# DavidPeicho/loupiote

Measured on AMD Instinct MI355X. Metric: Mrays/s (+ ms/frame) at 1920×1080, 4 spp, Sponza; 1/2/4/8 GPU, higher is better.
Workload: dtype f32

## Files before the change

bindings/rust/loupiote_hip/src/ffi.rs:

```rust
#![allow(non_camel_case_types, non_upper_case_globals, dead_code)]
use std::os::raw::{c_char, c_int, c_uint, c_void};

pub const LPT_ABI_VERSION: u32 = 6;
pub const LPT_INVALID_INDEX: u32 = 0xFFFFFFFF;
pub const LPT_PUNCTUAL_POINT: u32 = 0;
pub const LPT_PUNCTUAL_SPOT: u32 = 1;
pub const LPT_PUNCTUAL_DIRECTIONAL: u32 = 2;
pub const LPT_ALPHA_OPAQUE: u32 = 0;
pub const LPT_ALPHA_MASK: u32 = 1;
pub const LPT_ACCEL_BUILD_HOST_SAH: u32 = 0;
pub const LPT_ACCEL_BUILD_GPU_LBVH: u32 = 1;
pub const LPT_UPLOAD_NO_TEXTURE_PAIRS: u32 = 0x100;
pub const LPT_COMM_ID_BYTES: u32 = 128;
pub const LPT_OK: c_int = 0;
pub const LPT_ERR_FILE_NOT_FOUND: c_int = 1;
pub const LPT_ERR_READBACK: c_int = 2;
pub const LPT_ERR_ACCEL_BUILD: c_int = 3;
pub const LPT_ERR_HIP: c_int = 4;
pub const LPT_ERR_RCCL: c_int = 5;
pub const LPT_ERR_INVALID_ARG: c_int = 6;
pub const LPT_BLIT_PATHTRACE: c_int = 0;
pub const LPT_BLIT_DENOISED: c_int = 1;
pub const LPT_BLIT_TEMPORAL: c_int = 2;
pub const LPT_BLIT_GBUFFER: c_int = 3;
// ... 8 lines not shown
pub const LPT_OPT_TAIL_LANES: c_int = 5;
pub const LPT_OPT_EXPERIMENT_BASE: c_int = 256;
pub const LPT_EXP_PIPE_RAYS: c_int = 0;
pub const LPT_EXP_REFILL: c_int = 1;
pub const LPT_EXP_TRACE_WAVES_PER_CU: c_int = 2;
pub const LPT_EXP_SHADE_BLOCKS_PER_CU: c_int = 3;
pub const LPT_EXP_PATH_WAVES_PER_CU: c_int = 4;
pub const LPT_EXP_PATH_REFILL: c_int = 5;
pub const LPT_EXP_OCC_CELL_MILLI: c_int = 6;
pub const LPT_EXP_STEP_BUDGET: c_int = 7;
pub const LPT_EXP_BUDGET_RAYS: c_int = 8;
pub const LPT_EXP_PACKET_QUADS: c_int = 9;
pub const LPT_EXP_SPLIT_RAYS: c_int = 10;
pub const LPT_EXP_BUDGET_SPLIT: c_int = 11;
pub const LPT_EXP_LANE_PHASE: c_int = 12;

#[repr(C)] pub struct lpt_device { _private: [u8; 0] }
#[repr(C)] pub struct lpt_scene { _private: [u8; 0] }
#[repr(C)] pub struct lpt_scene_gpu { _private: [u8; 0] }
#[repr(C)] pub struct lpt_probe { _private: [u8; 0] }
#[repr(C)] pub struct lpt_renderer { _private: [u8; 0] }
#[repr(C)] pub struct lpt_comm { _private: [u8; 0] }
#[repr(C)] pub struct lpt_host_frame { _private: [u8; 0] }

#[repr(C)] #[derive(Copy, Clone, Debug)]
pub struct lpt_material {
    pub color: [f32; 4],
    pub roughness: f32,
    pub reflectivity: f32,
    pub albedo_texture: u32,
// ... 220 lines not shown
```

include/lpt.h:

```cpp
#ifndef LPT_H
#define LPT_H

#include <stddef.h>
#include <stdint.h>

#ifdef __cplusplus
extern "C" {
#endif

#define LPT_ABI_VERSION 6u

#define LPT_INVALID_INDEX 0xFFFFFFFFu

enum {
    LPT_OK = 0,
    LPT_ERR_FILE_NOT_FOUND = 1,
    LPT_ERR_READBACK = 2,
    LPT_ERR_ACCEL_BUILD = 3,
    LPT_ERR_HIP = 4,
    LPT_ERR_RCCL = 5,
    LPT_ERR_INVALID_ARG = 6
};

const char *lpt_last_error(void);
// ... 274 lines not shown
} lpt_option;
#define LPT_OPT_EXPERIMENT(name) (LPT_OPT_EXPERIMENT_BASE + (name))
typedef enum lpt_experiment {
    LPT_EXP_PIPE_RAYS = 0,
    LPT_EXP_REFILL = 1,
    LPT_EXP_TRACE_WAVES_PER_CU = 2,
    LPT_EXP_SHADE_BLOCKS_PER_CU = 3,
    LPT_EXP_PATH_WAVES_PER_CU = 4,
    LPT_EXP_PATH_REFILL = 5,
    LPT_EXP_OCC_CELL_MILLI = 6,
    LPT_EXP_STEP_BUDGET = 7,
    LPT_EXP_BUDGET_RAYS = 8,
    LPT_EXP_PACKET_QUADS = 9,
    LPT_EXP_SPLIT_RAYS = 10,
    LPT_EXP_BUDGET_SPLIT = 11,
    LPT_EXP_LANE_PHASE = 12
} lpt_experiment;
int lpt_renderer_set_option(lpt_renderer *r, int option, uint64_t value);
int lpt_renderer_get_option(const lpt_renderer *r, int option, uint64_t *value);
int lpt_shard_layout(uint32_t width, uint32_t height, uint32_t tile_w, uint32_t tile_h, uint32_t world_size, uint32_t rank,
                     uint32_t *out_slots, uint32_t *out_slot_offset);
int lpt_shard_layout_weighted(uint32_t width, uint32_t height, uint32_t tile_w, uint32_t tile_h, uint32_t world_size, uint32_t rank,
                              const uint32_t *weights_or_null, uint32_t *out_slots, uint32_t *out_slot_offset);
int lpt_shard_owner(uint32_t world_size, const uint32_t *weights_or_null, uint32_t tile, uint32_t *out_rank);
int lpt_renderer_get_ray_counts(lpt_renderer *r, lpt_ray_counts *out);
int lpt_renderer_get_queue_counts(lpt_renderer *r, uint32_t *closest, uint32_t *shadow, uint32_t cap);
int lpt_renderer_reset_ray_counts(lpt_renderer *r);
int lpt_renderer_get_step_histogram(lpt_renderer *r, uint32_t *max_steps, uint32_t *hist12);
int lpt_renderer_enable_stats(lpt_renderer *r, int flag);
int lpt_renderer_synchronize(lpt_renderer *r);
int lpt_renderer_stream(lpt_renderer *r, void **hip_stream);
// ... 6 lines not shown
```

loupiote_amd/_abi.py:

```python
import ctypes as C
import os

import numpy as np

_HERE = os.path.dirname(os.path.abspath(__file__))
LIB_PATH = os.environ.get("LPT_LIB_PATH") or os.path.join(_HERE, "libloupiote_hip.so")

LPT_OK = 0
LPT_ERR_FILE_NOT_FOUND = 1
LPT_ERR_READBACK = 2
LPT_ERR_ACCEL_BUILD = 3
LPT_ERR_HIP = 4
LPT_ERR_RCCL = 5
LPT_ERR_INVALID_ARG = 6
COMM_ID_BYTES = 128
OPT_EXPERIMENT_BASE = 256
OPTIONS = {"packet_primary": 1, "wavefront_rays": 2, "path_rays": 3, "coop_rays": 4, "tail_lanes": 5}
EXPERIMENTS = {"pipe_rays": 0, "refill": 1, "trace_waves_per_cu": 2, "shade_blocks_per_cu": 3, "path_waves_per_cu": 4, "path_refill": 5, "occ_cell_milli": 6,
               "step_budget": 7, "budget_rays": 8, "packet_quads": 9, "split_rays": 10, "budget_split": 11, "lane_phase": 12}
OPTIONS.update({k: OPT_EXPERIMENT_BASE + v for k, v in EXPERIMENTS.items()})
EXCHANGE_GATHER_TILES = 0
HOST_FRAME_HOST_ONLY = 1
EXCHANGE_REDUCE = 1
INVALID_INDEX = 0xFFFFFFFF
LIGHT_BIT = 0x80000000

MATERIAL_DT = np.dtype([("color", "<f4", 4), ("roughness", "<f4"), ("reflectivity", "<f4"),
                        ("albedo_texture", "<u4"), ("mra_texture", "<u4")])
VERTEX_DT = np.dtype([("position", "<f4", 4), ("normal", "<f4", 4)])
LIGHT_DT = np.dtype([("normal", "<f4", 4), ("tangent", "<f4", 4), ("bitangent", "<f4", 4), ("origin", "<f4", 4)])
PUNCTUAL_DT = np.dtype([("position", "<f4", 4), ("direction", "<f4", 4), ("color", "<f4", 4), ("cone", "<f4", 4)])
PUNCTUAL_POINT, PUNCTUAL_SPOT, PUNCTUAL_DIRECTIONAL = 0, 1, 2
ALPHA_OPAQUE, ALPHA_MASK = 0, 1
INSTANCE_DT = np.dtype([("model_to_world", "<f4", 16), ("blas_index", "<u4"), ("material_index", "<u4"),
# ... 181 lines not shown
```

loupiote_amd/csrc/device.hip:

```cpp
#include <hip/hip_runtime.h>

#include <dlfcn.h>

#include <algorithm>
#include <cmath>
#include <map>
#include <memory>
#include <cstdlib>
#include <functional>
#include <mutex>
#include <new>
#include <numeric>

#include "common.h"
#include "env_dist.h"
#include "kernels.h"
#include "build_kernels.h"
#include <hipcub/hipcub.hpp>
#include <rccl/rccl.h>

using namespace lpt;
using namespace lptd;

#define TRY(expr) do { const int st__ = (expr); if (st__ != LPT_OK) return st__; } while (0)
// ... 171 lines not shown
    uint32_t max_bounces = 3, user_seed = 0;
    int env_sampling = 0;
    float vfov = 0.78539816339744830962f;
    uint32_t rank = 0, world = 1, tile_w = 32, tile_h = 8;
    std::vector<uint32_t> weights;
    ShardMap map{1u, 1u, {0u}};
    ShardTable h_table{};
    std::vector<uint32_t> h_offset;
    ShardTable *d_table = nullptr;
    bool use_noise = false, stats = false, timings = false;
    int refill = 44;
    int sort_queues = 0;
    uint32_t shade_blocks_per_cu = 0;
    uint32_t trace_waves_per_cu = 0;
    uint32_t lane_phase = 1;
    uint32_t n_slots = 0;
    float4 *accum = nullptr, *scratch = nullptr;
    lpt_comm *comm = nullptr;
    float4 *frame = nullptr, *xstage = nullptr;
    size_t xstage_elems = 0;
    bool presented = false;
    hipEvent_t xevent = nullptr;
    bool xevent_recorded = false;
    Totals *totals = nullptr;
    uint32_t step_budget = kStepBudget, budget_rays = kBudgetRays;
    bool budget_split = false;
    uint32_t coop_rays = kCoopRays;
    uint32_t tail_lanes = 4u;
    uint64_t split_rays = kSplitRays;
    uint32_t *err_host = nullptr, *err_dev = nullptr;
// ... 1032 lines not shown
    HIP_TRY(hipMalloc(&wf.sq.o, sizeof(float4) * n));
    HIP_TRY(hipMalloc(&wf.sq.d, sizeof(float4) * n));
    HIP_TRY(hipMalloc(&wf.sq.c, sizeof(float4) * n));
    HIP_TRY(hipMalloc(&wf.hits, sizeof(float4) * n));
    HIP_TRY(hipMalloc(&wf.Lsum, sizeof(float4) * n));
    HIP_TRY(hipMalloc(&wf.strag, sizeof(uint32_t) * 2 * n));
    wf.ray_cap = n;
    return LPT_OK;
}

static int ensure_lane(lpt_renderer *r, int l) {
    Wavefront &wf = r->wf[l];
    if (l > 0 && !wf.stream) HIP_TRY(hipStreamCreateWithFlags(&wf.stream, hipStreamNonBlocking));
    if (!wf.done) HIP_TRY(hipEventCreateWithFlags(&wf.done, hipEventDisableTiming));
    if (!wf.consumed) HIP_TRY(hipEventCreateWithFlags(&wf.consumed, hipEventDisableTiming));
    if (!wf.ctr) HIP_TRY(hipMalloc(&wf.ctr, sizeof(FrameCounters)));
    return LPT_OK;
}

static int alloc_frame_buffers(lpt_renderer *r) {
    HIP_TRY(hipSetDevice(r->dev->ordinal));
    HIP_TRY(hipStreamSynchronize(r->stream));
    free_frame_buffers(r);
    if (!r->w || !r->h) return LPT_OK;
    uint32_t tiles_x, n_tiles, n_slots;
    shard_geometry(r, tiles_x, n_tiles, n_slots);
    const size_t px = (size_t)r->w * r->h;
    r->n_slots = n_slots;
    if (r->rank == 0u) {
        r->h_table = make_shard_table(r->weights, r->world, n_tiles, r->tile_w * r->tile_h, r->h_offset);
        if (!r->d_table) HIP_TRY(hipMalloc(&r->d_table, sizeof(ShardTable)));
// ... 257 lines not shown
    case LPT_OPT_EXPERIMENT(LPT_EXP_PIPE_RAYS): r->pipe_rays = (uint32_t)std::min<uint64_t>(value, 0x7FFFFFFFu); break;
    case LPT_OPT_WAVEFRONT_RAYS: r->wavefront_rays = std::max<uint64_t>(value, 64u); break;
    case LPT_OPT_EXPERIMENT(LPT_EXP_REFILL): if (value > 63u) return fail(LPT_ERR_INVALID_ARG, "LPT_EXP_REFILL: 0..63"); r->refill = (int)value; break;
    case LPT_OPT_EXPERIMENT(LPT_EXP_TRACE_WAVES_PER_CU): if (value > 32u) return fail(LPT_ERR_INVALID_ARG, "LPT_EXP_TRACE_WAVES_PER_CU: 0 (auto) or 1..32"); r->trace_waves_per_cu = (uint32_t)value; break;
    case LPT_OPT_EXPERIMENT(LPT_EXP_SHADE_BLOCKS_PER_CU): if (value > 64u) return fail(LPT_ERR_INVALID_ARG, "LPT_EXP_SHADE_BLOCKS_PER_CU: 0 (by the submission) or 1..64"); r->shade_blocks_per_cu = (uint32_t)value; break;
    case LPT_OPT_PATH_RAYS: r->path_rays = (uint32_t)std::min<uint64_t>(value, 0x7FFFFFFFu); break;
    case LPT_OPT_EXPERIMENT(LPT_EXP_PATH_WAVES_PER_CU): if (value < 1u || value > 32u) return fail(LPT_ERR_INVALID_ARG, "LPT_EXP_PATH_WAVES_PER_CU: 1..32"); r->path_waves_per_cu = (uint32_t)value; break;
    case LPT_OPT_EXPERIMENT(LPT_EXP_PATH_REFILL): if (value > 63u) return fail(LPT_ERR_INVALID_ARG, "LPT_EXP_PATH_REFILL: 0..63"); r->path_refill = (int)value; break;
    case LPT_OPT_EXPERIMENT(LPT_EXP_OCC_CELL_MILLI): r->occ_cell = (float)std::min<uint64_t>(value, 1000000u) * 1.0e-3f; break;
    case LPT_OPT_EXPERIMENT(LPT_EXP_STEP_BUDGET): r->step_budget = (uint32_t)std::min<uint64_t>(value, 1u << 20); break;
    case LPT_OPT_EXPERIMENT(LPT_EXP_BUDGET_RAYS): r->budget_rays = (uint32_t)std::min<uint64_t>(value, 0x7FFFFFFFu); break;
    case LPT_OPT_EXPERIMENT(LPT_EXP_PACKET_QUADS): r->packet_quads = value != 0; break;
    case LPT_OPT_EXPERIMENT(LPT_EXP_SPLIT_RAYS): r->split_rays = value; break;
    case LPT_OPT_EXPERIMENT(LPT_EXP_BUDGET_SPLIT): r->budget_split = value != 0; break;
    case LPT_OPT_EXPERIMENT(LPT_EXP_LANE_PHASE): if (value > 2u) return fail(LPT_ERR_INVALID_ARG, "LPT_EXP_LANE_PHASE: 0 (free), 1 (offset start), 2 (alternating traversal)"); r->lane_phase = (uint32_t)value; break;
    case LPT_OPT_TAIL_LANES: r->tail_lanes = (uint32_t)std::min<uint64_t>(value, kTailMax); break;
    case LPT_OPT_COOP_RAYS: r->coop_rays = (uint32_t)std::min<uint64_t>(value, 0x7FFFFFFFu); break;
    default: return fail(LPT_ERR_INVALID_ARG, "lpt_renderer_set_option: unknown option %d", option);
    }
    return LPT_OK;
}
int lpt_renderer_get_option(const lpt_renderer *r, int option, uint64_t *value) {
    if (!r || !value) return fail(LPT_ERR_INVALID_ARG, "lpt_renderer_get_option: null");
    switch (option) {
    case LPT_OPT_PACKET_PRIMARY: *value = r->packet_primary; break;
    case LPT_OPT_EXPERIMENT(LPT_EXP_PIPE_RAYS): *value = r->pipe_rays; break;
    case LPT_OPT_WAVEFRONT_RAYS: *value = r->wavefront_rays; break;
    case LPT_OPT_EXPERIMENT(LPT_EXP_REFILL): *value = (uint64_t)r->refill; break;
    case LPT_OPT_EXPERIMENT(LPT_EXP_TRACE_WAVES_PER_CU): *value = r->trace_waves_per_cu; break;
    case LPT_OPT_EXPERIMENT(LPT_EXP_SHADE_BLOCKS_PER_CU): *value = r->shade_blocks_per_cu; break;
    case LPT_OPT_PATH_RAYS: *value = r->path_rays; break;
    case LPT_OPT_EXPERIMENT(LPT_EXP_PATH_WAVES_PER_CU): *value = r->path_waves_per_cu; break;
    case LPT_OPT_EXPERIMENT(LPT_EXP_PATH_REFILL): *value = (uint64_t)r->path_refill; break;
    case LPT_OPT_EXPERIMENT(LPT_EXP_OCC_CELL_MILLI): *value = (uint64_t)(r->occ_cell * 1000.0f + 0.5f); break;
    case LPT_OPT_EXPERIMENT(LPT_EXP_STEP_BUDGET): *value = r->step_budget; break;
    case LPT_OPT_EXPERIMENT(LPT_EXP_BUDGET_RAYS): *value = r->budget_rays; break;
    case LPT_OPT_EXPERIMENT(LPT_EXP_PACKET_QUADS): *value = r->packet_quads; break;
    case LPT_OPT_EXPERIMENT(LPT_EXP_SPLIT_RAYS): *value = r->split_rays; break;
    case LPT_OPT_EXPERIMENT(LPT_EXP_BUDGET_SPLIT): *value = r->budget_split; break;
    case LPT_OPT_EXPERIMENT(LPT_EXP_LANE_PHASE): *value = r->lane_phase; break;
    case LPT_OPT_TAIL_LANES: *value = r->tail_lanes; break;
    case LPT_OPT_COOP_RAYS: *value = r->coop_rays; break;
    default: return fail(LPT_ERR_INVALID_ARG, "lpt_renderer_get_option: unknown option %d", option);
    }
    return LPT_OK;
}
int lpt_renderer_enable_stats(lpt_renderer *r, int flag) {
    if (!r) return fail(LPT_ERR_INVALID_ARG, "lpt_renderer_enable_stats: null");
    FLUSH_OR_RETURN(r);
    r->stats = flag != 0;
    if (flag) {
        HIP_TRY(hipSetDevice(r->dev->ordinal));
        if (!r->occ_table) HIP_TRY(hipMalloc(&r->occ_table, sizeof(uint32_t) * kOccEntries));
        HIP_TRY(hipMemsetAsync(r->occ_table, 0, sizeof(uint32_t) * kOccEntries, r->stream));
        HIP_TRY(hipStreamSynchronize(r->stream));
// ... 183 lines not shown
        const uint32_t trace_blocks = std::min<uint32_t>(div_up(n_rays, kTraceBlock), waves);
        const size_t lds = stack_bytes(sc);
        const bool dense = (r->w % r->tile_w == 0u) && (r->h % r->tile_h == 0u);

        const float pixel_rad = 2.0f * th / (float)std::max(r->h, 1u);
        const bool packet = !masked && (r->packet_primary == 1u || (r->packet_primary == 2u && pixel_rad <= kPacketMaxPixelRad));
        tk.packet = packet;
        OccProbe occ{nullptr, 0u, 0.0f};
        if (!masked && r->stats && r->occ_table && r->occ_cell > 0.0f) occ = OccProbe{r->occ_table, kOccEntries - 1u, 1.0f / r->occ_cell};
        const bool tail_launch = !masked && !r->stats && (solo || r->budget_split) && n_rays <= r->budget_rays;
        const uint32_t tail = tail_launch ? std::min(std::min(r->tail_lanes, kTailMax), (uint32_t)std::max(r->refill, 0)) : 0u;
        const uint32_t budget = (tail_launch && !tail && r->step_budget) ? r->step_budget : 0u;
        const size_t tail_lds = tail ? sizeof(uint32_t) * tail_lds_words(r->sg->stats.max_depth) : 0u;
        const bool coop_all = !masked && !r->stats && r->coop_rays && n_rays <= r->coop_rays;
        const bool path = !masked && r->path_rays && n_rays <= r->path_rays && !coop_all;
        const int slot = cur_slot(r);
        Wavefront *w = &wf;
        tk.stages = nb + 1u;
        tk.run = [=](uint32_t t, const PhaseHooks &ph) -> int {
            if (ph.wait_start) HIP_TRY(hipStreamWaitEvent(s, ph.wait_start, 0));
            auto trace = [&](int cb, int sb) {
                stage_begin(r, cb >= 0 ? ST_INTERSECT : ST_SHADOW, s, slot);
                const Queue qin = w->q[(uint32_t)(cb < 0 ? 0 : cb) & 1u];
                const int launch_no = cb >= 0 ? cb : (int)nb;
                if (coop_all) {
                    const size_t clds = sizeof(uint32_t) * coop_stack_entries(kCoopStack, r->sg->stats.max_depth);
                    hipLaunchKernelGGL(k_trace_coop<false>, dim3(std::min(2u * n_rays, cus * kCoopWavesPerCu)), dim3(kTraceBlock), clds, s, sc, qin, w->hits, w->sq, w->Lsum, w->ctr, cb, sb, (const uint32_t *)nullptr, launch_no);
                    stage_end(r, s, slot);
                    return;
                }
// ... 7 lines not shown
                    if (pipe) hipLaunchKernelGGL((k_trace<false, true, true>), dim3(trace_blocks), dim3(kTraceBlock), lds + tail_lds, s, TraceKernargs{sc, qin, w->hits, w->sq, w->Lsum, w->ctr, cb, sb, r->refill, occ, 0u, w->strag, launch_no, tail});
                    else hipLaunchKernelGGL((k_trace<false, false, true>), dim3(trace_blocks), dim3(kTraceBlock), lds + tail_lds, s, TraceKernargs{sc, qin, w->hits, w->sq, w->Lsum, w->ctr, cb, sb, r->refill, occ, 0u, w->strag, launch_no, tail});
                } else if (pipe) {
                    if (r->stats) hipLaunchKernelGGL((k_trace<true, true>), dim3(trace_blocks), dim3(kTraceBlock), lds + 64u, s, TraceKernargs{sc, qin, w->hits, w->sq, w->Lsum, w->ctr, cb, sb, r->refill, occ, budget, w->strag, launch_no, 0u});
                    else hipLaunchKernelGGL((k_trace<false, true>), dim3(trace_blocks), dim3(kTraceBlock), lds, s, TraceKernargs{sc, qin, w->hits, w->sq, w->Lsum, w->ctr, cb, sb, r->refill, occ, budget, w->strag, launch_no, 0u});
                } else if (r->stats) hipLaunchKernelGGL((k_trace<true, false>), dim3(trace_blocks), dim3(kTraceBlock), lds + 64u, s, TraceKernargs{sc, qin, w->hits, w->sq, w->Lsum, w->ctr, cb, sb, r->refill, occ, budget, w->strag, launch_no, 0u});
                else hipLaunchKernelGGL((k_trace<false, false>), dim3(trace_blocks), dim3(kTraceBlock), lds, s, TraceKernargs{sc, qin, w->hits, w->sq, w->Lsum, w->ctr, cb, sb, r->refill, occ, budget, w->strag, launch_no, 0u});
                if (budget) {
                    const size_t clds = sizeof(uint32_t) * coop_stack_entries(kCoopStack, r->sg->stats.max_depth);
                    if (r->stats) hipLaunchKernelGGL(k_trace_coop<true>, dim3(cus * kCoopWavesPerCu), dim3(kTraceBlock), clds, s, sc, qin, w->hits, w->sq, w->Lsum, w->ctr, cb, sb, w->strag, launch_no);
                    else hipLaunchKernelGGL(k_trace_coop<false>, dim3(cus * kCoopWavesPerCu), dim3(kTraceBlock), clds, s, sc, qin, w->hits, w->sq, w->Lsum, w->ctr, cb, sb, w->strag, launch_no);
                }
                stage_end(r, s, slot);
            };
            if (t == 0u) {
                HIP_TRY(hipMemsetAsync(w->ctr, 0, sizeof(FrameCounters), s));
                stage_begin(r, ST_RAYGEN, s, slot);
                if (dense) {
                    hipLaunchKernelGGL(k_raygen<true>, dim3(stream_blocks), dim3(kBlock), 0, s, p, nz, w->q[0], w->Lsum, w->ctr);
                } else {
                    hipLaunchKernelGGL(k_raygen<false>, dim3(stream_blocks), dim3(kBlock), 0, s, p, nz, w->q[0], w->Lsum, w->ctr);
                }
                stage_end(r, s, slot);
                if (ph.wait_trav) HIP_TRY(hipStreamWaitEvent(s, ph.wait_trav, 0));
                if (packet) {
                    stage_begin(r, ST_PRIMARY, s, slot);
                    const uint32_t packets = div_up(n_rays, 64u);
                    const size_t plds = (size_t)(48u + 7u * r->sg->stats.max_depth + 8u) * sizeof(uint32_t);
                    const uint32_t quad_slots = (r->packet_quads && dense && p.block8 && p.n_slots % 64u == 0u && p.slot0 % 64u == 0u && n_samples % 4u == 0u) ? p.n_slots : 0u;
                    if (r->stats) hipLaunchKernelGGL(k_trace_packet<true>, dim3(std::min(packets, cus * kPacketBlocksPerCu)), dim3(kTraceBlock), plds, s, sc, w->q[0], w->hits, w->ctr, 0, quad_slots);
                    else hipLaunchKernelGGL(k_trace_packet<false>, dim3(std::min(packets, cus * kPacketBlocksPerCu)), dim3(kTraceBlock), plds, s, sc, w->q[0], w->hits, w->ctr, 0, quad_slots);
                    stage_end(r, s, slot);
                } else if (coop_all || !path) trace(0, -1);
                if (path) {
                    stage_begin(r, ST_PATH, s, slot);
                    const uint32_t pblocks = std::min<uint32_t>(div_up(n_rays, kTraceBlock), std::max(8u, (cus * r->path_waves_per_cu) & ~7u));
                    const size_t plds = lds + kPathLdsExtra;
                    auto launch_path = [&](auto G, auto S, auto P) {
                        constexpr bool g = decltype(G)::value, st = decltype(S)::value, pu = decltype(P)::value;
                        const float4 *h0 = packet ? w->hits : (const float4 *)nullptr;
                        if (env) hipLaunchKernelGGL((k_path<g, st, true, pu, DEnv>), dim3(pblocks), dim3(kTraceBlock), plds, s, sc, probe, nz, p, w->q[0], h0, w->Lsum, w->ctr, seed0, gb, r->path_refill, ev);
                        else hipLaunchKernelGGL((k_path<g, st, false, pu>), dim3(pblocks), dim3(kTraceBlock), plds, s, sc, probe, nz, p, w->q[0], h0, w->Lsum, w->ctr, seed0, gb, r->path_refill);
                    };
                    auto path_gs = [&](auto P) {
                        if (denoise) { if (r->stats) launch_path(std::true_type{}, std::true_type{}, P); else launch_path(std::true_type{}, std::false_type{}, P); }
                        else if (r->stats) launch_path(std::false_type{}, std::true_type{}, P);
                        else launch_path(std::false_type{}, std::false_type{}, P);
                    };
                    if (punct) path_gs(std::true_type{}); else path_gs(std::false_type{});
                    stage_end(r, s, slot);
                }
            } else if (!path) {
                const uint32_t b = t - 1u;
                const uint32_t seed = seed0 + t;
                const Queue qin = w->q[b & 1u], qout = w->q[(b + 1u) & 1u];
                stage_begin(r, ST_SHADE, s, slot);
                auto launch_shade = [&](auto G, auto P) {
                    constexpr bool g = decltype(G)::value, pu = decltype(P)::value;
                    if (env) hipLaunchKernelGGL((k_shade<g, true, pu, DEnv>), dim3(shade_blocks), dim3(kBlock), 0, s, sc, probe, nz, p, qin, w->hits, qout, w->sq, w->Lsum, w->ctr, (int)b, seed, gb, r->sort_queues, ev);
                    else hipLaunchKernelGGL((k_shade<g, false, pu>), dim3(shade_blocks), dim3(kBlock), 0, s, sc, probe, nz, p, qin, w->hits, qout, w->sq, w->Lsum, w->ctr, (int)b, seed, gb, r->sort_queues);
                };
                if (denoise && b == 0u) { if (punct) launch_shade(std::true_type{}, std::true_type{}); else launch_shade(std::true_type{}, std::false_type{}); }
                else if (punct) launch_shade(std::false_type{}, std::true_type{});
                else launch_shade(std::false_type{}, std::false_type{});
                stage_end(r, s, slot);
                if (ph.wait_trav) HIP_TRY(hipStreamWaitEvent(s, ph.wait_trav, 0));
                trace(b + 1u < nb ? (int)(b + 1u) : -1, (int)b);
            }
            if (ph.rec_trav) HIP_TRY(hipEventRecord(ph.rec_trav, s));
            if (t == nb && split) HIP_TRY(hipEventRecord(w->done, s));
            HIP_TRY(hipGetLastError());
            return LPT_OK;
        };
        for (uint32_t t = 0; !defer && t < tk.stages; ++t) {
            const int st = tk.run(t, PhaseHooks{});
            if (st != LPT_OK) return st;
        }
// ... 766 lines not shown
```

loupiote_amd/csrc/kernels.h:

```cpp
#pragma once
#include "device_math.h"

namespace lptd {

constexpr int kMaxBounces = 64;
constexpr int kBlock = 256;
constexpr int kTraceBlock = 64;

struct DNode8 {
    uint4 n0;
    uint4 n2;
    uint4 n3;
    uint4 n4;
};
using lpt::kNodeTris;

__device__ __forceinline__ uint32_t node_imask(const uint4 &n0) { return (n0.z >> 8) & 0xFFu; }
__device__ __forceinline__ uint32_t node_leaves(const uint4 &n0) { return n0.z >> 16; }
__device__ __forceinline__ uint32_t leaf_count(uint32_t V, uint32_t slot) { return 1u + ((V >> (8u + slot)) & 1u); }
struct NodeGrid { float px, py, pz, sx, sy, sz; };
template <typename Scene>
__device__ __forceinline__ NodeGrid node_grid(const Scene &sc, const uint4 &n0) {
    NodeGrid g;
    g.px = fmaf((float)(n0.x & 0xFFFFu), sc.grid_step[0], sc.grid_lo[0]);
// ... 199 lines not shown

__device__ __forceinline__ void noise_shift(const DNoise &nz, uint32_t x, uint32_t y, uint32_t seed_counter, float &r0, float &r1) {
    if (!nz.enabled) return;
    const uint8_t *t = nz.rgba + 4u * ((size_t)(y % nz.h) * nz.w + (x % nz.w));
    float g = (float)(seed_counter & 1023u) * 0.61803398875f;
    float a = r0 + ((float)t[0] + 0.5f) * 0.00390625f + g;
    float b = r1 + ((float)t[1] + 0.5f) * 0.00390625f + g;
    a = a - floorf(a);
    b = b - floorf(b);
    if (a >= 1.0f) a = 0.0f;
    if (b >= 1.0f) b = 0.0f;
    r0 = a;
    r1 = b;
}

template <bool DENSE>
__global__ __launch_bounds__(kBlock) void k_raygen(FrameParams p, DNoise nz, Queue q, float4 *Lsum, FrameCounters *ctr) {
    __shared__ uint32_t lds[8];
    const uint32_t stride = gridDim.x * blockDim.x;
    const uint32_t total = p.n_slots * p.n_samples;
    const uint32_t rounded = (total + (kBlock - 1u)) & ~(uint32_t)(kBlock - 1u);
    if (DENSE && blockIdx.x == 0 && threadIdx.x == 0) QC(ctr, 0) = total;
    for (uint32_t vslot = blockIdx.x * blockDim.x + threadIdx.x; vslot < rounded; vslot += stride) {
        const uint32_t sample = vslot / p.n_slots, slot = vslot - sample * p.n_slots;
        const uint32_t seed_counter = p.seed_counter + sample * p.max_bounces;
        uint32_t x = 0, y = 0;
        const bool valid = vslot < total && slot_to_pixel(p, p.slot0 + slot, x, y);
        if (vslot < total) Lsum[vslot] = make_float4(0.f, 0.f, 0.f, 0.f);
        f3 d = mk3(0.f, 0.f, 0.f);
        if (valid) {
            const uint32_t pixel = y * p.width + x;
            Rng r = rng_init(pixel, stage_seed(p.user_seed, seed_counter), LPT_TAG_RAYGEN);
            float jx = rng_next(r), jy = rng_next(r);
            noise_shift(nz, x, y, seed_counter, jx, jy);
            float sx = ((float)x + jx) / (float)p.width;
            float sy = ((float)y + jy) / (float)p.height;
            float cx = (2.0f * sx - 1.0f) * p.ax;
            float cy = (1.0f - 2.0f * sy) * p.ay;
            f3 dir = mk3((p.right.x * cx + p.up.x * cy) + p.fwd.x, (p.right.y * cx + p.up.y * cy) + p.fwd.y,
                         (p.right.z * cx + p.up.z * cy) + p.fwd.z);
            d = normalize(dir);
        }
        const uint32_t idx = DENSE ? vslot : block_compact(valid, &QC(ctr, 0), lds);
        if (valid) {
            st_nt(q.o + idx, make_float4(p.origin.x, p.origin.y, p.origin.z, -1.0f));
            st_nt(q.d + idx, make_float4(d.x, d.y, d.z, __uint_as_float(vslot)));
            q.T[idx] = make_float4(1.f, 1.f, 1.f, __uint_as_float(x | (y << 13) | (sample << 26)));
        }
    }
}

struct Hit { float t, u, v; uint32_t prim; };

__device__ __forceinline__ bool ray_triangle(const float4 r0, const float4 r1, const float4 r2, f3 o, f3 d, float tmax, float &t, float &u, float &v) {
    float oz = fmaf(r2.z, o.z, fmaf(r2.y, o.y, fmaf(r2.x, o.x, r2.w)));
    float dz = fmaf(r2.z, d.z, fmaf(r2.y, d.y, r2.x * d.x));
    float tt = -oz / dz;
    if (!(tt > 0.0f && tt <= tmax)) return false;
    float ox = fmaf(r0.z, o.z, fmaf(r0.y, o.y, fmaf(r0.x, o.x, r0.w)));
    float dx = fmaf(r0.z, d.z, fmaf(r0.y, d.y, r0.x * d.x));
    float uu = fmaf(tt, dx, ox);
    if (!(uu >= 0.0f)) return false;
// ... 678 lines not shown
typedef uint32_t u32x4 __attribute__((ext_vector_type(4)));
__device__ __forceinline__ void sload_node_header(const void *p, uint4 &a) {
    u32x4 va;
    asm volatile("s_load_dwordx4 %0, %1, 0x0\n\ts_waitcnt lgkmcnt(0)" : "=&s"(va) : "s"(p) : "memory");
    a = make_uint4(va.x, va.y, va.z, va.w);
}
__device__ __forceinline__ void sload_tri(const void *p, float4 &a, float4 &b, float4 &c) {
    u32x4 va, vb, vc;
    asm volatile("s_load_dwordx4 %0, %3, 0x0\n\ts_load_dwordx4 %1, %3, 0x10\n\ts_load_dwordx4 %2, %3, 0x20\n\ts_waitcnt lgkmcnt(0)"
                 : "=&s"(va), "=&s"(vb), "=&s"(vc) : "s"(p) : "memory");
    a = make_float4(__uint_as_float(va.x), __uint_as_float(va.y), __uint_as_float(va.z), __uint_as_float(va.w));
    b = make_float4(__uint_as_float(vb.x), __uint_as_float(vb.y), __uint_as_float(vb.z), __uint_as_float(vb.w));
    c = make_float4(__uint_as_float(vc.x), __uint_as_float(vc.y), __uint_as_float(vc.z), __uint_as_float(vc.w));
}

template <bool STATS>
__global__ __launch_bounds__(kTraceBlock) __attribute__((amdgpu_waves_per_eu(8))) void k_trace_packet(DScene sc, Queue q, float4 *hits, FrameCounters *ctr, int bounce, uint32_t quad_slots) {
    static_assert(kTraceBlock == 64, "k_trace_packet: planes[] and stk[] are per-wave LDS, the block must be one wave");
    float *planes = reinterpret_cast<float *>(lds_dyn);
    uint32_t *stk = reinterpret_cast<uint32_t *>(lds_dyn) + 48;
    const DNode8 *__restrict__ nodes = sc.nodes;
    const float4 *__restrict__ woop = sc.woop;
    const uint32_t *__restrict__ leaf_prim = sc.leaf_prim;
    const uint32_t count = QC(ctr, bounce);
    const uint32_t lane = threadIdx.x;
    uint32_t visits = 0, tests = 0;
    for (uint32_t base = blockIdx.x * 64u; base < count; base += gridDim.x * 64u) {
        uint32_t ray = base + lane;
        if (quad_slots) {
            const uint32_t pk = base >> 6;
            const uint32_t blocks = quad_slots >> 6;
            const uint32_t grp = pk / (blocks * 4u), rem = pk - grp * (blocks * 4u);
            const uint32_t blk = rem >> 2, qtr = rem & 3u;
            const uint32_t smp = grp * 4u + (lane >> 4), sub = lane & 15u;
            const uint32_t px = (qtr & 1u) * 4u + (sub & 3u), py = (qtr >> 1) * 4u + (sub >> 2);
            ray = smp * quad_slots + blk * 64u + py * 8u + px;
        }
        const bool live = ray < count;
        f3 o = mk3(0.f, 0.f, 0.f), d = mk3(0.f, 0.f, 1.f);
        if (live) { const float4 o4 = q.o[ray], d4 = q.d[ray]; o = mk3(o4.x, o4.y, o4.z); d = mk3(d4.x, d4.y, d4.z); }
        const float ix = safe_inv(d.x), iy = safe_inv(d.y), iz = safe_inv(d.z);
        const bool negx = ix < 0.0f, negy = iy < 0.0f, negz = iz < 0.0f;
        Hit best;
        best.t = live ? LPT_T_INF : -1.0f; best.u = 0.f; best.v = 0.f; best.prim = 0xFFFFFFFFu;
        const uint32_t onx = negx ? 24u : 0u, ofx = negx ? 0u : 24u, ony = negy ? 32u : 8u, ofy = negy ? 8u : 32u, onz = negz ? 40u : 16u, ofz = negz ? 16u : 40u;
        const uint32_t oinv = (uint32_t)__builtin_amdgcn_readfirstlane((int)(7u - ((negx ? 1u : 0u) | (negy ? 2u : 0u) | (negz ? 4u : 0u))));
        const unsigned long long lv = __ballot(live);
        const int l0 = lv ? __ffsll((long long)lv) - 1 : 0;
        const float o0x = __uint_as_float((uint32_t)__builtin_amdgcn_readlane((int)__float_as_uint(o.x), l0)), o0y = __uint_as_float((uint32_t)__builtin_amdgcn_readlane((int)__float_as_uint(o.y), l0)),
                    o0z = __uint_as_float((uint32_t)__builtin_amdgcn_readlane((int)__float_as_uint(o.z), l0));
        const bool coherent = lv != 0ull && __ballot(live && (o.x != o0x || o.y != o0y || o.z != o0z)) == 0ull &&
                              ((__ballot(live && negx) == 0ull) || (__ballot(live && negx) == lv)) && ((__ballot(live && negy) == 0ull) || (__ballot(live && negy) == lv)) &&
                              ((__ballot(live && negz) == 0ull) || (__ballot(live && negz) == lv));
        float ixlo = live ? ix : 3.0e38f, ixhi = live ? ix : -3.0e38f, iylo = live ? iy : 3.0e38f, iyhi = live ? iy : -3.0e38f, izlo = live ? iz : 3.0e38f, izhi = live ? iz : -3.0e38f;
#pragma unroll
// ... 85 lines not shown
            for (uint32_t m = inner; m; m &= m - 1u) keyed |= 1u << (((uint32_t)__ffs((int)m) - 1u) ^ oinv);
            for (uint32_t m = keyed; m; m &= m - 1u) {
                const uint32_t sl = ((uint32_t)__ffs((int)m) - 1u) ^ oinv;
                const uint32_t rel = (uint32_t)__popc(imask & ~(0xFFFFFFFFu << sl));
                if (lane == 0) stk[sp] = n0.w + rel;
                sp++;
            }
            have = sp > 0;
            __syncthreads();
            if (have) { sp--; node_index = (uint32_t)__builtin_amdgcn_readfirstlane((int)stk[sp]); }
        }
        if (live) {
            intersect_lights(sc, o, d, best);
            st_nt(hits + ray, make_float4(best.t, best.u, best.v, __uint_as_float(best.prim)));
        }
    }
    if (STATS && lane == 0) {
        atomicAdd(&ctr->packet_nodes, (unsigned long long)visits);
        atomicAdd(&ctr->packet_tris, (unsigned long long)tests);
    }
}

template <bool MASK = false>
__global__ __launch_bounds__(kTraceBlock) void k_query_closest(DScene sc, const float4 *o, const float4 *d, float4 *hits, uint32_t n) {
    uint2 *stack = reinterpret_cast<uint2 *>(lds_dyn) + threadIdx.x;
    const uint32_t i = blockIdx.x * blockDim.x + threadIdx.x;
    if (i >= n) return;
    const float4 o4 = o[i], d4 = d[i];
    const f3 oo = mk3(o4.x, o4.y, o4.z), dd = mk3(d4.x, d4.y, d4.z);
    Hit h;
    uint32_t a = 0, b = 0;
// ... 463 lines not shown
        }
    }
    if (GBUF && bounce == 0) {
        const uint32_t gx = pxy & 0x1FFFu, gy = (pxy >> 13) & 0x1FFFu;
        const size_t px = (size_t)gy * p.width + gx;
        gb.gbuf[px] = make_uint4(prim, __float_as_uint(h4.x), oct_encode(g_n), pack_albedo(g_alb));
        float mu = 0.0f, mv = 0.0f, cu, cv, pu, pv;
        if (prim != 0xFFFFFFFFu && project(gb.cur, g_P, cu, cv) && project(gb.prev, g_P, pu, pv)) { mu = pu - cu; mv = pv - cv; }
        gb.motion[px] = make_float2(mu, mv);
    }
}

#ifndef LPT_SHADE_WAVES
#define LPT_SHADE_WAVES(ENV, PUNCT) (((ENV) || (PUNCT)) ? 3 : 4)
#endif
template <bool GBUF, bool ENV = false, bool PUNCT = false, typename... Env>
__global__ __launch_bounds__(kBlock) __attribute__((amdgpu_waves_per_eu(LPT_SHADE_WAVES(ENV, PUNCT)))) void k_shade(DScene sc, DProbe probe, DNoise nz, FrameParams p, Queue qin, const float4 *hits,
                                                  Queue qout, ShadowQueue sq, float4 *Lsum, FrameCounters *ctr, int bounce,
                                                  uint32_t seed_base, GBufArgs gb, int sorted, Env... env) {
    static_assert(sizeof...(Env) == (ENV ? 1u : 0u), "the ENV instantiations take the distribution, the others nothing");
    const DEnv ev = env_arg(env...);
    __shared__ uint32_t lds[72];
    __shared__ float s_lut[256];
    __shared__ float4 s_park[6 * kBlock];
    __shared__ uint32_t s_at[2 * kBlock];
    s_lut[threadIdx.x] = sc.srgb_lut[threadIdx.x];
    __syncthreads();
    bool parked = false;
    const uint32_t count = QC(ctr, bounce);
    const uint32_t stride = gridDim.x * blockDim.x;
    const uint32_t rounded = (count + 255u) & ~255u;
    uint32_t n_surface = 0;
    const bool last_bounce = (uint32_t)bounce + 1u >= p.max_bounces;
    const PunctPick pk = PUNCT ? punct_pick<ENV>(sc) : PunctPick{0.0f, 0.0f};
    const float inv_nl = rect_inv_nl<ENV, PUNCT>(sc, pk);
    for (uint32_t i0 = blockIdx.x * blockDim.x + threadIdx.x; i0 < rounded; i0 += stride) {
        ShadeOut so;
        so.want_next = false; so.want_shadow = false; so.is_surface = false;
        const uint32_t i = i0;
        if (i < count) {
            const float4 d4 = ld_nt(qin.d + i), T4 = ld_nt(qin.T + i), h4 = ld_nt(hits + i);
            const uint32_t slot = __float_as_uint(d4.w);
            shade_hit<GBUF, ENV, PUNCT>(sc, probe, ev, nz, p, s_lut, (uint32_t)bounce, last_bounce, seed_base, inv_nl, pk, gb, d4, T4, h4,
                            [&]() { return ld_nt(qin.o + i); },
                            [&](float r, float g, float b) {
                                float4 L = Lsum[slot];
                                L.x = L.x + r; L.y = L.y + g; L.z = L.z + b;
                                Lsum[slot] = L;
                            }, so);
        }
        if (!(sorted & 3)) {
            const bool va = so.want_shadow, vb = so.want_next && !last_bounce;
            const unsigned long long ma = __ballot(va), mb = __ballot(vb);
            const uint32_t lane = threadIdx.x & 63u, wave = threadIdx.x >> 6;
            const unsigned long long lt = (1ull << lane) - 1ull;
            const uint32_t wa = (uint32_t)__popcll(ma & lt), wb = (uint32_t)__popcll(mb & lt);
            if (!parked && i0 + stride < rounded) {
                if (lane == 0) lds[16 + wave] = (uint32_t)__popcll(ma) | ((uint32_t)__popcll(mb) << 16);
                s_at[threadIdx.x] = va ? wa : 0xFFFFFFFFu;
// ... 409 lines not shown

__global__ __launch_bounds__(kBlock) void k_debug_view(const uint4 *gb, const float2 *motion, uchar4 *out, int W, int H, int mode) {
    const uint32_t i = blockIdx.x * blockDim.x + threadIdx.x;
    if (i >= (uint32_t)(W * H)) return;
    if (mode == 3) {
        const f3 n = oct_decode(gb[i].z);
        out[i] = make_uchar4((uint8_t)((n.x * 0.5f + 0.5f) * 255.0f + 0.5f), (uint8_t)((n.y * 0.5f + 0.5f) * 255.0f + 0.5f),
                             (uint8_t)((n.z * 0.5f + 0.5f) * 255.0f + 0.5f), 255);
    } else {
        const float2 m = motion[i];
        out[i] = make_uchar4((uint8_t)(clampf(fabsf(m.x) * (float)W * 0.125f, 0.0f, 1.0f) * 255.0f + 0.5f),
                             (uint8_t)(clampf(fabsf(m.y) * (float)H * 0.125f, 0.0f, 1.0f) * 255.0f + 0.5f), 0, 255);
    }
}

__global__ __launch_bounds__(64) void k_finish_frame(FrameCounters *ctr, Totals *tot, uint32_t bounces, uint32_t packet_primary) {
    static_assert(kMaxBounces <= 64, "a lane per bounce");
    if (blockIdx.x != 0) return;
    const uint32_t b = threadIdx.x;
    unsigned long long c = 0, s = 0, sh = 0;
    if (b < bounces) {
        c = QC(ctr, (int)b); s = SC(ctr, (int)b); sh = ctr->shaded[b];
        for (uint32_t k = 0; k < 8u; ++k) sh += ctr->shaded_part[(b * 8u + k) * 32u];
    }
#pragma unroll
    for (int off = 32; off > 0; off >>= 1) { c += __shfl_xor(c, off); s += __shfl_xor(s, off); sh += __shfl_xor(sh, off); }
    if (b != 0) return;
    if (packet_primary) { tot->primary += QC(ctr, 0); tot->packet_nodes += ctr->packet_nodes; tot->packet_tris += ctr->packet_tris; }
    tot->closest += c; tot->shadow += s; tot->shaded += sh; tot->nodes += ctr->nodes; tot->tris += ctr->tris;
    tot->shadow_nodes += ctr->shadow_nodes; tot->shadow_tris += ctr->shadow_tris;
// ... 185 lines not shown
```

Before: 6384.

## Fuse primary ray generation into packet trace and primary shade kernels

Adds an on-by-default fuse_primary path. When packet tracing is dense and not in path, coop or denoise mode, the separate raygen kernel is skipped. The packet trace kernel generates each primary ray inline and zeroes Lsum, and the bounce-0 shade kernel regenerates direction and throughput instead of loading them from the queue. The full FrameCounters memset is also replaced by a kernel that only clears the rows for bounces in use. This removes one launch and the queue writes and reads for primary rays, at the cost of recomputing ray generation twice and launching one block per packet.

```diff
diff --git a/bindings/rust/loupiote_hip/src/ffi.rs b/bindings/rust/loupiote_hip/src/ffi.rs
--- a/bindings/rust/loupiote_hip/src/ffi.rs
+++ b/bindings/rust/loupiote_hip/src/ffi.rs
@@ -46,6 +46,7 @@
 pub const LPT_EXP_SPLIT_RAYS: c_int = 10;
 pub const LPT_EXP_BUDGET_SPLIT: c_int = 11;
 pub const LPT_EXP_LANE_PHASE: c_int = 12;
+pub const LPT_EXP_FUSE_PRIMARY: c_int = 13;
 
 #[repr(C)] pub struct lpt_device { _private: [u8; 0] }
 #[repr(C)] pub struct lpt_scene { _private: [u8; 0] }
diff --git a/include/lpt.h b/include/lpt.h
--- a/include/lpt.h
+++ b/include/lpt.h
@@ -312,7 +312,8 @@
     LPT_EXP_PACKET_QUADS = 9,
     LPT_EXP_SPLIT_RAYS = 10,
     LPT_EXP_BUDGET_SPLIT = 11,
-    LPT_EXP_LANE_PHASE = 12
+    LPT_EXP_LANE_PHASE = 12,
+    LPT_EXP_FUSE_PRIMARY = 13
 } lpt_experiment;
 int lpt_renderer_set_option(lpt_renderer *r, int option, uint64_t value);
 int lpt_renderer_get_option(const lpt_renderer *r, int option, uint64_t *value);
diff --git a/loupiote_amd/_abi.py b/loupiote_amd/_abi.py
--- a/loupiote_amd/_abi.py
+++ b/loupiote_amd/_abi.py
@@ -17,7 +17,7 @@
 OPT_EXPERIMENT_BASE = 256
 OPTIONS = {"packet_primary": 1, "wavefront_rays": 2, "path_rays": 3, "coop_rays": 4, "tail_lanes": 5}
 EXPERIMENTS = {"pipe_rays": 0, "refill": 1, "trace_waves_per_cu": 2, "shade_blocks_per_cu": 3, "path_waves_per_cu": 4, "path_refill": 5, "occ_cell_milli": 6,
-               "step_budget": 7, "budget_rays": 8, "packet_quads": 9, "split_rays": 10, "budget_split": 11, "lane_phase": 12}
+               "step_budget": 7, "budget_rays": 8, "packet_quads": 9, "split_rays": 10, "budget_split": 11, "lane_phase": 12, "fuse_primary": 13}
 OPTIONS.update({k: OPT_EXPERIMENT_BASE + v for k, v in EXPERIMENTS.items()})
 EXCHANGE_GATHER_TILES = 0
 HOST_FRAME_HOST_ONLY = 1
diff --git a/loupiote_amd/csrc/device.hip b/loupiote_amd/csrc/device.hip
--- a/loupiote_amd/csrc/device.hip
+++ b/loupiote_amd/csrc/device.hip
@@ -209,6 +209,7 @@
     uint32_t shade_blocks_per_cu = 0;
     uint32_t trace_waves_per_cu = 0;
     uint32_t lane_phase = 1;
+    bool fuse_primary = true;
     uint32_t n_slots = 0;
     float4 *accum = nullptr, *scratch = nullptr;
     lpt_comm *comm = nullptr;
@@ -1271,7 +1272,10 @@
     if (l > 0 && !wf.stream) HIP_TRY(hipStreamCreateWithFlags(&wf.stream, hipStreamNonBlocking));
     if (!wf.done) HIP_TRY(hipEventCreateWithFlags(&wf.done, hipEventDisableTiming));
     if (!wf.consumed) HIP_TRY(hipEventCreateWithFlags(&wf.consumed, hipEventDisableTiming));
-    if (!wf.ctr) HIP_TRY(hipMalloc(&wf.ctr, sizeof(FrameCounters)));
+    if (!wf.ctr) {
+        HIP_TRY(hipMalloc(&wf.ctr, sizeof(FrameCounters)));
+        HIP_TRY(hipMemset(wf.ctr, 0, sizeof(FrameCounters)));
+    }
     return LPT_OK;
 }
 
@@ -1559,6 +1563,7 @@
     case LPT_OPT_EXPERIMENT(LPT_EXP_SPLIT_RAYS): r->split_rays = value; break;
     case LPT_OPT_EXPERIMENT(LPT_EXP_BUDGET_SPLIT): r->budget_split = value != 0; break;
     case LPT_OPT_EXPERIMENT(LPT_EXP_LANE_PHASE): if (value > 2u) return fail(LPT_ERR_INVALID_ARG, "LPT_EXP_LANE_PHASE: 0 (free), 1 (offset start), 2 (alternating traversal)"); r->lane_phase = (uint32_t)value; break;
+    case LPT_OPT_EXPERIMENT(LPT_EXP_FUSE_PRIMARY): r->fuse_primary = value != 0; break;
     case LPT_OPT_TAIL_LANES: r->tail_lanes = (uint32_t)std::min<uint64_t>(value, kTailMax); break;
     case LPT_OPT_COOP_RAYS: r->coop_rays = (uint32_t)std::min<uint64_t>(value, 0x7FFFFFFFu); break;
     default: return fail(LPT_ERR_INVALID_ARG, "lpt_renderer_set_option: unknown option %d", option);
@@ -1584,6 +1589,7 @@
     case LPT_OPT_EXPERIMENT(LPT_EXP_SPLIT_RAYS): *value = r->split_rays; break;
     case LPT_OPT_EXPERIMENT(LPT_EXP_BUDGET_SPLIT): *value = r->budget_split; break;
     case LPT_OPT_EXPERIMENT(LPT_EXP_LANE_PHASE): *value = r->lane_phase; break;
+    case LPT_OPT_EXPERIMENT(LPT_EXP_FUSE_PRIMARY): *value = r->fuse_primary; break;
     case LPT_OPT_TAIL_LANES: *value = r->tail_lanes; break;
     case LPT_OPT_COOP_RAYS: *value = r->coop_rays; break;
     default: return fail(LPT_ERR_INVALID_ARG, "lpt_renderer_get_option: unknown option %d", option);
@@ -1797,6 +1803,7 @@
         const size_t tail_lds = tail ? sizeof(uint32_t) * tail_lds_words(r->sg->stats.max_depth) : 0u;
         const bool coop_all = !masked && !r->stats && r->coop_rays && n_rays <= r->coop_rays;
         const bool path = !masked && r->path_rays && n_rays <= r->path_rays && !coop_all;
+        const bool fused = r->fuse_primary && packet && dense && !path && !coop_all && !denoise;
         const int slot = cur_slot(r);
         Wavefront *w = &wf;
         tk.stages = nb + 1u;
@@ -1834,22 +1841,30 @@
                 stage_end(r, s, slot);
             };
             if (t == 0u) {
-                HIP_TRY(hipMemsetAsync(w->ctr, 0, sizeof(FrameCounters), s));
-                stage_begin(r, ST_RAYGEN, s, slot);
-                if (dense) {
-                    hipLaunchKernelGGL(k_raygen<true>, dim3(stream_blocks), dim3(kBlock), 0, s, p, nz, w->q[0], w->Lsum, w->ctr);
-                } else {
-                    hipLaunchKernelGGL(k_raygen<false>, dim3(stream_blocks), dim3(kBlock), 0, s, p, nz, w->q[0], w->Lsum, w->ctr);
+                hipLaunchKernelGGL(k_clear_counters, dim3(std::min(8u, nb)), dim3(kBlock), 0, s, w->ctr, nb);
+                if (!fused) {
+                    stage_begin(r, ST_RAYGEN, s, slot);
+                    if (dense) {
+                        hipLaunchKernelGGL(k_raygen<true>, dim3(stream_blocks), dim3(kBlock), 0, s, p, nz, w->q[0], w->Lsum, w->ctr);
+                    } else {
+                        hipLaunchKernelGGL(k_raygen<false>, dim3(stream_blocks), dim3(kBlock), 0, s, p, nz, w->q[0], w->Lsum, w->ctr);
+                    }
+                    stage_end(r, s, slot);
                 }
-                stage_end(r, s, slot);
                 if (ph.wait_trav) HIP_TRY(hipStreamWaitEvent(s, ph.wait_trav, 0));
                 if (packet) {
                     stage_begin(r, ST_PRIMARY, s, slot);
                     const uint32_t packets = div_up(n_rays, 64u);
                     const size_t plds = (size_t)(48u + 7u * r->sg->stats.max_depth + 8u) * sizeof(uint32_t);
                     const uint32_t quad_slots = (r->packet_quads && dense && p.block8 && p.n_slots % 64u == 0u && p.slot0 % 64u == 0u && n_samples % 4u == 0u) ? p.n_slots : 0u;
-                    if (r->stats) hipLaunchKernelGGL(k_trace_packet<true>, dim3(std::min(packets, cus * kPacketBlocksPerCu)), dim3(kTraceBlock), plds, s, sc, w->q[0], w->hits, w->ctr, 0, quad_slots);
-                    else hipLaunchKernelGGL(k_trace_packet<false>, dim3(std::min(packets, cus * kPacketBlocksPerCu)), dim3(kTraceBlock), plds, s, sc, w->q[0], w->hits, w->ctr, 0, quad_slots);
+                    const dim3 pgrid(std::min(packets, cus * kPacketBlocksPerCu));
+                    if (fused) {
+                        const PrimaryGen gen{p, nz, w->Lsum, n_rays};
+                        const dim3 ggrid(packets);
+                        if (r->stats) hipLaunchKernelGGL((k_trace_packet<true, true, PrimaryGen>), ggrid, dim3(kTraceBlock), plds, s, sc, w->q[0], w->hits, w->ctr, 0, quad_slots, gen);
+                        else hipLaunchKernelGGL((k_trace_packet<false, true, PrimaryGen>), ggrid, dim3(kTraceBlock), plds, s, sc, w->q[0], w->hits, w->ctr, 0, quad_slots, gen);
+                    } else if (r->stats) hipLaunchKernelGGL(k_trace_packet<true>, pgrid, dim3(kTraceBlock), plds, s, sc, w->q[0], w->hits, w->ctr, 0, quad_slots);
+                    else hipLaunchKernelGGL(k_trace_packet<false>, pgrid, dim3(kTraceBlock), plds, s, sc, w->q[0], w->hits, w->ctr, 0, quad_slots);
                     stage_end(r, s, slot);
                 } else if (coop_all || !path) trace(0, -1);
                 if (path) {
@@ -1877,10 +1892,16 @@
                 stage_begin(r, ST_SHADE, s, slot);
                 auto launch_shade = [&](auto G, auto P) {
                     constexpr bool g = decltype(G)::value, pu = decltype(P)::value;
-                    if (env) hipLaunchKernelGGL((k_shade<g, true, pu, DEnv>), dim3(shade_blocks), dim3(kBlock), 0, s, sc, probe, nz, p, qin, w->hits, qout, w->sq, w->Lsum, w->ctr, (int)b, seed, gb, r->sort_queues, ev);
+                    if (env) hipLaunchKernelGGL((k_shade<g, true, pu, false, DEnv>), dim3(shade_blocks), dim3(kBlock), 0, s, sc, probe, nz, p, qin, w->hits, qout, w->sq, w->Lsum, w->ctr, (int)b, seed, gb, r->sort_queues, ev);
                     else hipLaunchKernelGGL((k_shade<g, false, pu>), dim3(shade_blocks), dim3(kBlock), 0, s, sc, probe, nz, p, qin, w->hits, qout, w->sq, w->Lsum, w->ctr, (int)b, seed, gb, r->sort_queues);
                 };
-                if (denoise && b == 0u) { if (punct) launch_shade(std::true_type{}, std::true_type{}); else launch_shade(std::true_type{}, std::false_type{}); }
+                auto launch_primary = [&](auto P) {
+                    constexpr bool pu = decltype(P)::value;
+                    if (env) hipLaunchKernelGGL((k_shade<false, true, pu, true, DEnv>), dim3(shade_blocks), dim3(kBlock), 0, s, sc, probe, nz, p, qin, w->hits, qout, w->sq, w->Lsum, w->ctr, (int)b, seed, gb, r->sort_queues, ev);
+                    else hipLaunchKernelGGL((k_shade<false, false, pu, true>), dim3(shade_blocks), dim3(kBlock), 0, s, sc, probe, nz, p, qin, w->hits, qout, w->sq, w->Lsum, w->ctr, (int)b, seed, gb, r->sort_queues);
+                };
+                if (fused && b == 0u) { if (punct) launch_primary(std::true_type{}); else launch_primary(std::false_type{}); }
+                else if (denoise && b == 0u) { if (punct) launch_shade(std::true_type{}, std::true_type{}); else launch_shade(std::true_type{}, std::false_type{}); }
                 else if (punct) launch_shade(std::false_type{}, std::true_type{});
                 else launch_shade(std::false_type{}, std::false_type{});
                 stage_end(r, s, slot);
diff --git a/loupiote_amd/csrc/kernels.h b/loupiote_amd/csrc/kernels.h
--- a/loupiote_amd/csrc/kernels.h
+++ b/loupiote_amd/csrc/kernels.h
@@ -237,6 +237,33 @@
     r1 = b;
 }
 
+struct PrimaryRay { uint32_t x, y, sample; f3 d; bool valid; };
+__device__ __forceinline__ PrimaryRay primary_ray(const FrameParams &p, const DNoise &nz, uint32_t vslot) {
+    PrimaryRay pr;
+    pr.sample = vslot / p.n_slots;
+    const uint32_t slot = vslot - pr.sample * p.n_slots;
+    const uint32_t seed_counter = p.seed_counter + pr.sample * p.max_bounces;
+    pr.x = 0; pr.y = 0;
+    pr.d = mk3(0.f, 0.f, 0.f);
+    pr.valid = slot_to_pixel(p, p.slot0 + slot, pr.x, pr.y);
+    if (pr.valid) {
+        const uint32_t x = pr.x, y = pr.y;
+        const uint32_t pixel = y * p.width + x;
+        Rng r = rng_init(pixel, stage_seed(p.user_seed, seed_counter), LPT_TAG_RAYGEN);
+        float jx = rng_next(r), jy = rng_next(r);
+        noise_shift(nz, x, y, seed_counter, jx, jy);
+        float sx = ((float)x + jx) / (float)p.width;
+        float sy = ((float)y + jy) / (float)p.height;
+        float cx = (2.0f * sx - 1.0f) * p.ax;
+        float cy = (1.0f - 2.0f * sy) * p.ay;
+        f3 dir = mk3((p.right.x * cx + p.up.x * cy) + p.fwd.x, (p.right.y * cx + p.up.y * cy) + p.fwd.y,
+                     (p.right.z * cx + p.up.z * cy) + p.fwd.z);
+        pr.d = normalize(dir);
+    }
+    return pr;
+}
+__device__ __forceinline__ uint32_t primary_pxy(const PrimaryRay &pr) { return pr.x | (pr.y << 13) | (pr.sample << 26); }
+
 template <bool DENSE>
 __global__ __launch_bounds__(kBlock) void k_raygen(FrameParams p, DNoise nz, Queue q, float4 *Lsum, FrameCounters *ctr) {
     __shared__ uint32_t lds[8];
@@ -245,30 +272,18 @@
     const uint32_t rounded = (total + (kBlock - 1u)) & ~(uint32_t)(kBlock - 1u);
     if (DENSE && blockIdx.x == 0 && threadIdx.x == 0) QC(ctr, 0) = total;
     for (uint32_t vslot = blockIdx.x * blockDim.x + threadIdx.x; vslot < rounded; vslot += stride) {
-        const uint32_t sample = vslot / p.n_slots, slot = vslot - sample * p.n_slots;
-        const uint32_t seed_counter = p.seed_counter + sample * p.max_bounces;
-        uint32_t x = 0, y = 0;
-        const bool valid = vslot < total && slot_to_pixel(p, p.slot0 + slot, x, y);
-        if (vslot < total) Lsum[vslot] = make_float4(0.f, 0.f, 0.f, 0.f);
-        f3 d = mk3(0.f, 0.f, 0.f);
-        if (valid) {
-            const uint32_t pixel = y * p.width + x;
-            Rng r = rng_init(pixel, stage_seed(p.user_seed, seed_counter), LPT_TAG_RAYGEN);
-            float jx = rng_next(r), jy = rng_next(r);
-            noise_shift(nz, x, y, seed_counter, jx, jy);
-            float sx = ((float)x + jx) / (float)p.width;
-            float sy = ((float)y + jy) / (float)p.height;
-            float cx = (2.0f * sx - 1.0f) * p.ax;
-            float cy = (1.0f - 2.0f * sy) * p.ay;
-            f3 dir = mk3((p.right.x * cx + p.up.x * cy) + p.fwd.x, (p.right.y * cx + p.up.y * cy) + p.fwd.y,
-                         (p.right.z * cx + p.up.z * cy) + p.fwd.z);
-            d = normalize(dir);
-        }
+        PrimaryRay pr;
+        pr.valid = false;
+        if (vslot < total) {
+            pr = primary_ray(p, nz, vslot);
+            Lsum[vslot] = make_float4(0.f, 0.f, 0.f, 0.f);
+        }
+        const bool valid = pr.valid;
         const uint32_t idx = DENSE ? vslot : block_compact(valid, &QC(ctr, 0), lds);
         if (valid) {
             st_nt(q.o + idx, make_float4(p.origin.x, p.origin.y, p.origin.z, -1.0f));
-            st_nt(q.d + idx, make_float4(d.x, d.y, d.z, __uint_as_float(vslot)));
-            q.T[idx] = make_float4(1.f, 1.f, 1.f, __uint_as_float(x | (y << 13) | (sample << 26)));
+            st_nt(q.d + idx, make_float4(pr.d.x, pr.d.y, pr.d.z, __uint_as_float(vslot)));
+            q.T[idx] = make_float4(1.f, 1.f, 1.f, __uint_as_float(primary_pxy(pr)));
         }
     }
 }
@@ -977,18 +992,28 @@
     c = make_float4(__uint_as_float(vc.x), __uint_as_float(vc.y), __uint_as_float(vc.z), __uint_as_float(vc.w));
 }
 
-template <bool STATS>
-__global__ __launch_bounds__(kTraceBlock) __attribute__((amdgpu_waves_per_eu(8))) void k_trace_packet(DScene sc, Queue q, float4 *hits, FrameCounters *ctr, int bounce, uint32_t quad_slots) {
+struct PrimaryGen { FrameParams p; DNoise nz; float4 *Lsum; uint32_t count; };
+__device__ __forceinline__ const PrimaryGen *gen_arg() { return nullptr; }
+__device__ __forceinline__ const PrimaryGen *gen_arg(const PrimaryGen &g) { return &g; }
+template <bool STATS, bool GEN = false, typename... Gen>
+__global__ __launch_bounds__(kTraceBlock) __attribute__((amdgpu_waves_per_eu(8))) void k_trace_packet(DScene sc, Queue q, float4 *hits, FrameCounters *ctr, int bounce, uint32_t quad_slots, Gen... gen) {
+    static_assert(sizeof...(Gen) == (GEN ? 1u : 0u), "the GEN instantiations take the frame's parameters, the others nothing");
+    const PrimaryGen *gp = gen_arg(gen...);
     static_assert(kTraceBlock == 64, "k_trace_packet: planes[] and stk[] are per-wave LDS, the block must be one wave");
     float *planes = reinterpret_cast<float *>(lds_dyn);
     uint32_t *stk = reinterpret_cast<uint32_t *>(lds_dyn) + 48;
     const DNode8 *__restrict__ nodes = sc.nodes;
     const float4 *__restrict__ woop = sc.woop;
     const uint32_t *__restrict__ leaf_prim = sc.leaf_prim;
-    const uint32_t count = QC(ctr, bounce);
     const uint32_t lane = threadIdx.x;
+    uint32_t count;
+    if constexpr (GEN) {
+        count = gp->count;
+        if (blockIdx.x == 0 && lane == 0) QC(ctr, bounce) = count;
+    } else count = QC(ctr, bounce);
     uint32_t visits = 0, tests = 0;
-    for (uint32_t base = blockIdx.x * 64u; base < count; base += gridDim.x * 64u) {
+    uint32_t base = blockIdx.x * 64u;
+    if (base < count) do {
         uint32_t ray = base + lane;
         if (quad_slots) {
             const uint32_t pk = base >> 6;
@@ -999,9 +1024,16 @@
             const uint32_t px = (qtr & 1u) * 4u + (sub & 3u), py = (qtr >> 1) * 4u + (sub >> 2);
             ray = smp * quad_slots + blk * 64u + py * 8u + px;
         }
-        const bool live = ray < count;
+        bool live = ray < count;
         f3 o = mk3(0.f, 0.f, 0.f), d = mk3(0.f, 0.f, 1.f);
-        if (live) { const float4 o4 = q.o[ray], d4 = q.d[ray]; o = mk3(o4.x, o4.y, o4.z); d = mk3(d4.x, d4.y, d4.z); }
+        if constexpr (GEN) {
+            if (live) {
+                gp->Lsum[ray] = make_float4(0.f, 0.f, 0.f, 0.f);
+                const PrimaryRay pr = primary_ray(gp->p, gp->nz, ray);
+                live = pr.valid;
+                if (live) { o = gp->p.origin; d = pr.d; }
+            }
+        } else if (live) { const float4 o4 = q.o[ray], d4 = q.d[ray]; o = mk3(o4.x, o4.y, o4.z); d = mk3(d4.x, d4.y, d4.z); }
         const float ix = safe_inv(d.x), iy = safe_inv(d.y), iz = safe_inv(d.z);
         const bool negx = ix < 0.0f, negy = iy < 0.0f, negz = iz < 0.0f;
         Hit best;
@@ -1117,7 +1149,7 @@
             intersect_lights(sc, o, d, best);
             st_nt(hits + ray, make_float4(best.t, best.u, best.v, __uint_as_float(best.prim)));
         }
-    }
+    } while (!GEN && (base += gridDim.x * 64u) < count);
     if (STATS && lane == 0) {
         atomicAdd(&ctr->packet_nodes, (unsigned long long)visits);
         atomicAdd(&ctr->packet_tris, (unsigned long long)tests);
@@ -1611,7 +1643,7 @@
 #ifndef LPT_SHADE_WAVES
 #define LPT_SHADE_WAVES(ENV, PUNCT) (((ENV) || (PUNCT)) ? 3 : 4)
 #endif
-template <bool GBUF, bool ENV = false, bool PUNCT = false, typename... Env>
+template <bool GBUF, bool ENV = false, bool PUNCT = false, bool PRIMARY = false, typename... Env>
 __global__ __launch_bounds__(kBlock) __attribute__((amdgpu_waves_per_eu(LPT_SHADE_WAVES(ENV, PUNCT)))) void k_shade(DScene sc, DProbe probe, DNoise nz, FrameParams p, Queue qin, const float4 *hits,
                                                   Queue qout, ShadowQueue sq, float4 *Lsum, FrameCounters *ctr, int bounce,
                                                   uint32_t seed_base, GBufArgs gb, int sorted, Env... env) {
@@ -1636,10 +1668,16 @@
         so.want_next = false; so.want_shadow = false; so.is_surface = false;
         const uint32_t i = i0;
         if (i < count) {
-            const float4 d4 = ld_nt(qin.d + i), T4 = ld_nt(qin.T + i), h4 = ld_nt(hits + i);
+            float4 d4, T4;
+            if constexpr (PRIMARY) {
+                const PrimaryRay pr = primary_ray(p, nz, i);
+                d4 = make_float4(pr.d.x, pr.d.y, pr.d.z, __uint_as_float(i));
+                T4 = make_float4(1.f, 1.f, 1.f, __uint_as_float(primary_pxy(pr)));
+            } else { d4 = ld_nt(qin.d + i); T4 = ld_nt(qin.T + i); }
+            const float4 h4 = ld_nt(hits + i);
             const uint32_t slot = __float_as_uint(d4.w);
             shade_hit<GBUF, ENV, PUNCT>(sc, probe, ev, nz, p, s_lut, (uint32_t)bounce, last_bounce, seed_base, inv_nl, pk, gb, d4, T4, h4,
-                            [&]() { return ld_nt(qin.o + i); },
+                            [&]() { return PRIMARY ? make_float4(p.origin.x, p.origin.y, p.origin.z, -1.0f) : ld_nt(qin.o + i); },
                             [&](float r, float g, float b) {
                                 float4 L = Lsum[slot];
                                 L.x = L.x + r; L.y = L.y + g; L.z = L.z + b;
@@ -2079,6 +2117,19 @@
     }
 }
 
+__global__ __launch_bounds__(kBlock) void k_clear_counters(FrameCounters *ctr, uint32_t bounces) {
+    constexpr uint32_t kWords = sizeof(FrameCounters) / 4u, kRow = 8u * 32u;
+    constexpr uint32_t i0 = offsetof(FrameCounters, ihead) / 4u, s0 = offsetof(FrameCounters, shead) / 4u, m0 = offsetof(FrameCounters, strag_count) / 4u,
+                       p0 = offsetof(FrameCounters, shaded_part) / 4u, p1 = p0 + kMaxBounces * kRow;
+    static_assert(sizeof(FrameCounters) % 4u == 0u && s0 == i0 + kMaxBounces * kRow && m0 == s0 + kMaxBounces * kRow, "k_clear_counters: the layout of FrameCounters");
+    uint32_t *w = reinterpret_cast<uint32_t *>(ctr);
+    const uint32_t rows = bounces * kRow, tid = blockIdx.x * blockDim.x + threadIdx.x, stride = gridDim.x * blockDim.x;
+    for (uint32_t k = tid; k < i0; k += stride) w[k] = 0u;
+    for (uint32_t k = tid; k < rows; k += stride) { w[i0 + k] = 0u; w[s0 + k] = 0u; w[p0 + k] = 0u; }
+    for (uint32_t k = m0 + tid; k < p0; k += stride) w[k] = 0u;
+    for (uint32_t k = p1 + tid; k < kWords; k += stride) w[k] = 0u;
+}
+
 __global__ __launch_bounds__(64) void k_finish_frame(FrameCounters *ctr, Totals *tot, uint32_t bounces, uint32_t packet_primary) {
     static_assert(kMaxBounces <= 64, "a lane per bounce");
     if (blockIdx.x != 0) return;
```

New measurement: 6439 (median of 6 runs). No clear change (+0.9%).
